# nianticlabs/implicit-depth

Hardware: AMD Instinct MI355X
Metric: frames/sec (BDModel.forward hot path, 512x384, 64 planes, 8-frame tuple = 1 current + 7 source views; third-party backbones excluded) (higher is better)
Workload: dtype f32

## Files before the change

### implicit-depth_amd/csrc/conv.hip

```cpp
#include <algorithm>
#include "conv_args.h"
#include "../../include/idh_ops.h"

using namespace idh_conv;

int idh_stem_op(const idh_op &op, hipStream_t st, bool launch);

namespace {

__device__ float g_zero_page[kZeroFloats];

thread_local bool t_dry_run = false;
thread_local int t_launches = 0;
#undef IDH_CHECK_LAUNCH
#define IDH_CHECK_LAUNCH()                                              \
    do {                                                                \
        if (!t_dry_run && hipGetLastError() != hipSuccess) return IDH_ELAUNCH; \
    } while (0)
#define IDH_LAUNCH(...)                         \
    do {                                        \
        if (t_dry_run) ++t_launches;            \
        else hipLaunchKernelGGL(__VA_ARGS__);   \
    } while (0)

// ... 1252 lines not shown
    } else {
        int tm = op.tile_m, tn = op.tile_n;
        if (tm == 8 || tm == 9) tm = 0;
        const int nsub = a.Cout_pad / 16;
        if (tn == 0) tn = (nsub % 4 == 0) ? 4 : (nsub % 2 == 0 ? 2 : 1);
        if (tm == 0) tm = 4;
        if ((tm != 1 && tm != 2 && tm != 4) || (tn != 1 && tn != 2 && tn != 4) || nsub % tn) return IDH_EINVAL;
        a.MT = (int)((M + 16 * tm - 1) / (16 * tm));
        a.NT = nsub / tn;
        pc.tm = tm; pc.tn = tn;
        const long long waves = (long long)a.MT * a.NT * a.S;
        if ((waves + 3) / 4 >= (1ll << 31)) return IDH_EUNSUPPORTED;
        pc.blocks = (unsigned)((waves + 3) / 4);
    }
    if (pc.up && ((pc.lds_rows != 8 && pc.lds_rows != 4) || pc.nj != 4)) return IDH_EUNSUPPORTED;
    if (pc.norm && ((pc.lds_rows != 8 && pc.lds_rows != 4) || pc.nj != 1)) return IDH_EUNSUPPORTED;
    if (a.S > 1) {
        if (!op.ws) return IDH_EWORKSPACE;
        pc.red = ReduceDesc{op.ws, op.bias, op.res, op.out, a.M, op.Cout, a.Cout_pad, a.S, op.res_cs, op.out_cs, op.act, op.slope};
    }
    return IDH_OK;
}

int launch_conv(const PreparedConv &pc, hipStream_t st) {
    if (pc.lds_rows == 16) {
        if (t_dry_run) { ++t_launches; return IDH_OK; }
        return launch_conv_split(pc.a, pc.n_img, pc.tm, pc.tn, st);
    }
    if (pc.lds_rows == 32) {
        if (t_dry_run) { ++t_launches; return IDH_OK; }
        return launch_conv_wino(pc.a, pc.n_img, pc.tn, st);
// ... 159 lines not shown
                    } else {
                        break;
                    }
                    ++run;
                }
                int cnt = 0;
                if (op.kind == IDH_OP_CONV && pcs[0].lds_rows == 4 && !pcs[0].norm && !pcs[0].s2) {
                    cnt = 1;
                    while (cnt < run && ops[i + cnt].kind == IDH_OP_CONV && pcs[cnt].lds_rows == 4 && pcs[cnt].nj == pcs[0].nj &&
                           (!pcs[cnt].up || pcs[0].nj == 4) && !pcs[cnt].norm && !pcs[cnt].s2)
                        ++cnt;
                }
                int mix = 0;
                while (mix < run && kinds[mix] >= 0 && pcs[mix].blocks <= kLevelMaxBlocks) ++mix;
                int wg = 0;
                if (op.kind == IDH_OP_CONV && pcs[0].lds_rows == 32) {
                    wg = 1;
                    while (wg < run && wg < wino_max_group() && ops[i + wg].kind == IDH_OP_CONV && pcs[wg].lds_rows == 32 &&
                           (pcs[wg].a.s[1].in != nullptr) == (pcs[0].a.s[1].in != nullptr))
                        ++wg;
                }
                int rc, used;
                if (wg > 1) {
                    if (t_dry_run) {
                        ++t_launches;
                        rc = IDH_OK;
                    } else {
                        const ConvArgs *as[kMaxGroup];
                        int ns[kMaxGroup];
                        for (int j = 0; j < wg; ++j) { as[j] = &pcs[j].a; ns[j] = pcs[j].n_img; }
                        rc = launch_conv_wino_group(as, ns, wg, st);
                        if (rc == IDH_EUNSUPPORTED) {
                            rc = IDH_OK;
// ... 176 lines not shown
```

### implicit-depth_amd/csrc/conv_wino.hip

```cpp
#include <type_traits>

#include "conv_args.h"
#include "../../include/idh_ops.h"

using namespace idh_conv;

namespace {

typedef unsigned u32x4_t __attribute__((ext_vector_type(4)));
typedef __attribute__((address_space(3))) void lds_void;

constexpr int kWinoCH = 8;
constexpr int kWinoTileW = 32;
constexpr int kWinoHalf = 17;
constexpr int kOob = 0x7fffffff;

constexpr int wino_plane(int WAVES) { return (2 * WAVES + 2) * 2 * kWinoHalf; }
constexpr int wino_qs(int WAVES) { return (wino_plane(WAVES) + 63) / 64 * 64; }
constexpr int wino_stage(int WAVES, int NCO) { return 4 * wino_qs(WAVES) + NCO * 1024; }

__global__ __launch_bounds__(256) void pack_wino_weight_k(const float *__restrict__ w, float *__restrict__ dst, int Cout, int Cin, int nS, int nCB, int KS) {
    const long long total = (long long)nS * nCB * 16 * 64 * KS;
    for (long long t = blockIdx.x * 256ll + threadIdx.x; t < total; t += gridDim.x * 256ll) {
        const int e = (int)(t % KS);
// ... 32 lines not shown
#endif

struct WinoArgs {
    ConvArgs c;
    int tiles_x, tiles_y;
    int tiles;
};

template <int WAVES, int NCO, int CH, bool SRC2>
constexpr int wino_stage_slots() {
    constexpr int halo = ((CH / 4) * wino_plane(WAVES) + 63) / 64 * 64;
    constexpr int s3 = halo + 64 * NCO * 4 * (CH / 4), sp = 8 * 32 * 2 * WAVES + 64 * 2 * NCO;
    return SRC2 && sp > s3 ? sp : s3;
}

template <int WAVES, int NCO, int CH, bool SRC2>
__device__ __forceinline__ void wino_tiles(const WinoArgs &wa, f32x4 *lds, const unsigned vblock, const unsigned vgrid) {
    constexpr int KS = CH / 4;
    constexpr int NP = CH / 4;
    typedef float vec __attribute__((ext_vector_type(KS)));
    constexpr int kRows = 2 * WAVES;
    constexpr int kPlane = wino_plane(WAVES);
    static_assert(NP == 2, "halo swizzle written for 8-channel K steps");
    constexpr int kHaloPieces = (NP * kPlane + 63) / 64;
    constexpr int kHP = (kHaloPieces + WAVES - 1) / WAVES;
    constexpr int kPanelPieces = NCO * 4 * KS;
    static_assert(kPanelPieces % WAVES == 0, "panel pieces must split evenly over the waves");
    constexpr int kPanel = kPanelPieces / WAVES;
    constexpr int kTPW = kHP + kPanel;
    static_assert(CH == 8, "K steps of 8 channels: every tile has >= 2 steps (the first stores the previous tile's outputs, the last loads the residual)");
    static_assert(kTPW <= 8 && 4 * NCO <= 8, "one DMA piece per even position group, one output store per odd group");
// ... 36 lines not shown
        unsigned blk = (unsigned)t;
        const int nt = blk % a.NT; blk /= a.NT;
        const int tx = blk % wa.tiles_x; blk /= wa.tiles_x;
        const int ty = blk % wa.tiles_y;
        img = blk / wa.tiles_y;
        y0 = ty * kRows; x0 = tx * kWinoTileW; cb0 = nt * NCO;
    };
    BufRef rsA;
    int voffH[kHP], panel_so;
    const int voffP = 16 * lane;
    auto halo_piece = [&](int k) { return wave + WAVES * k < kHaloPieces ? wave + WAVES * k : wave; };
    auto halo_voff = [&](int j, int lane) {
        const int pt = 32 * j + (lane >> 1);
        const int row = pt / kWinoHalf, hxh = pt - row * kWinoHalf;
        const int q = (lane & 1) ^ ((hxh >> 3) & 1);
        const int iy = y0 - 1 + (row >> 1), ix = x0 - 1 + 2 * hxh + (row & 1);
        const bool ok = (pt < kPlane) & ((unsigned)iy < (unsigned)s.H) & ((unsigned)ix < (unsigned)s.W);
        return ok ? (iy * s.W + ix) * s.cs * 4 + 16 * q : kOob;
    };
    auto set_fetch_tile = [&]() {
        rsA = BufRef{s.in + (size_t)img * s.H * s.W * s.cs, s.H * s.W * s.cs * 4};
        int lane_o = lane;
        asm volatile("" : "+v"(lane_o));
#pragma unroll
        for (int k = 0; k < kHP; ++k) voffH[k] = halo_voff(halo_piece(k), lane_o);
        panel_so = (cb0 * (4 * KS) + wave * kPanel) * 1024;
    };
    static_assert(!SRC2 || (kTight == 64 * WAVES && 2 * NCO == WAVES), "P-step pieces: eight of the pixels and one of the panel per wave");
    constexpr int kTPW2 = SRC2 ? 9 : 0;
    const ConvSrc &s1 = a.s[1];
    const int nS2 = SRC2 ? (s1.cblocks + 1) / 2 : 0;
// ... 42 lines not shown
                const int hh = wave / NCO, cbw = wave % NCO;
                halo1 = false;
                vo1 = voffP2; so1 = (4 * (2 * c + hh) * a.Cout_pad + 16 * (cbf + cbw)) * 16; lo1 = 8 * kTight + 64 * wave;
            }
            const int m = -(int)p;
            const unsigned long long m64 = (unsigned long long)(long long)m;
            vo ^= (vo ^ vo1) & m; so ^= (so ^ so1) & m; lo ^= (lo ^ lo1) & m;
            const BufRef rs1 = halo1 ? rsA2 : rsW2;
            const unsigned long long p0 = (unsigned long long)rs.p, p1 = (unsigned long long)rs1.p;
            rs.p = reinterpret_cast<const float *>(p0 ^ ((p0 ^ p1) & m64));
            rs.bytes ^= (rs.bytes ^ rs1.bytes) & m;
        }
        dma16(rs, lds + __builtin_amdgcn_readfirstlane(stage * kStage + lo), vo, __builtin_amdgcn_readfirstlane(so));
    };

    f32x4 acc[16][NCO];
    f32x4 ost[2][2][NCO];
    int voffS[2][2];
    __amdgpu_buffer_rsrc_t rsS;
    bool pending = false;

    const int pq = (KS * h) >> 2, pb8 = ((KS * h) & 3) * 4;
    const int patch0 = (NP * ((4 * wave) * kWinoHalf + n) + (pq ^ ((n >> 3) & 1))) * 16 + pb8;
    const int frag0 = kHalo * 16 + (h * 16 + n) * (4 * KS);

    constexpr int kAhead = CH == 16 ? 2 : 3;
    auto compute = [&](int stage, bool pnext, int cnext, int snext, int cbf, bool flush) {
        typedef const __attribute__((address_space(3))) volatile char lds_cchar;
        typedef const __attribute__((address_space(3))) volatile vec lds_cvec;
        int n_o = n;
        asm volatile("" : "+v"(n_o));
        const int patch1 = patch0 + (NP + ((pq ^ (((n_o + 1) >> 3) & 1)) - (pq ^ ((n_o >> 3) & 1)))) * 16;
        lds_cchar *sH0 = (lds_cchar *)(lds + stage * kStage) + patch0, *sH1 = (lds_cchar *)(lds + stage * kStage) + patch1;
        lds_cchar *sW = (lds_cchar *)(lds + stage * kStage) + frag0;
        vec d[4][4], A[kAhead + 1][NCO], r[4];
        auto rd_frag = [&](int g) {
            const int p = ((g >> 2) == 0 ? 4 : (g >> 2) == 1 ? 8 : (g >> 2) == 2 ? 0 : 12) + (g & 3);
#pragma unroll
            for (int j = 0; j < NCO; ++j) A[g % (kAhead + 1)][j] = *(lds_cvec *)(sW + (j * 16 + p) * 64 * (4 * KS));
        };
        auto rd_row = [&](int y) {
#pragma unroll
            for (int x = 0; x < 4; ++x) d[y][x] = *(lds_cvec *)(((x >> 1) ? sH1 : sH0) + NP * (2 * y + (x & 1)) * kWinoHalf * 16);
        };
        rd_frag(0);
        rd_row(1);
        rd_row(2);
#pragma unroll
        for (int g = 1; g < kAhead; ++g) rd_frag(g);
#pragma unroll
        for (int g = 0; g < 16; ++g) {
            const int xi = (g >> 2) == 0 ? 1 : (g >> 2) == 1 ? 2 : (g >> 2) == 2 ? 0 : 3, nu = g & 3;
            const int p = 4 * xi + nu;
            if (g + kAhead < 16) rd_frag(g + kAhead);
            if (g == 5) rd_row(0);
            if (g == 9) rd_row(3);
#ifndef IDH_ABL_WINO_NODMA
            if ((g & 1) == 0 && (g >> 1) < kTPW) issue_next(g >> 1, pnext, cnext, snext, cbf);
            if (SRC2 && (g == 1 || g == 3) && kTPW + (g >> 1) < kTPW2) {
// ... 2 lines not shown
#endif
#ifndef IDH_ABL_WINO_NOSTORE
            if ((g & 1) == 1 && (g >> 1) < 4 * NCO && flush) {
                const int k = g >> 1;
                __builtin_amdgcn_raw_buffer_store_b128(__builtin_bit_cast(u32x4_t, ost[k >> 1 & 1][k & 1][k >> 2]), rsS, voffS[k >> 1 & 1][k & 1] + 64 * (k >> 2), 0, 0);
            }
#endif
            __builtin_amdgcn_sched_barrier(0);
#ifdef IDH_ABL_WINO_SCALARXF
            auto vadd = [](vec a, vec b) { vec o; for (int e = 0; e < KS; ++e) { float t = a[e] + b[e]; asm("" : "+v"(t)); o[e] = t; } return o; };
            auto vsub = [](vec a, vec b) { vec o; for (int e = 0; e < KS; ++e) { float t = a[e] - b[e]; asm("" : "+v"(t)); o[e] = t; } return o; };
#else
            auto vadd = [](vec a, vec b) { return a + b; };
            auto vsub = [](vec a, vec b) { return a - b; };
#endif
#ifndef IDH_ABL_WINO_NOXFORM
            if (nu == 0) {
#pragma unroll
                for (int x = 0; x < 4; ++x)
                    r[x] = xi == 0 ? vsub(d[0][x], d[2][x]) : xi == 1 ? vadd(d[1][x], d[2][x]) : xi == 2 ? vsub(d[2][x], d[1][x]) : vsub(d[1][x], d[3][x]);
            }
#endif
#ifdef IDH_ABL_WINO_NOXFORM
            const vec v = d[xi][nu];
#else
            const vec v = nu == 0 ? vsub(r[0], r[2]) : nu == 1 ? vadd(r[1], r[2]) : nu == 2 ? vsub(r[2], r[1]) : vsub(r[1], r[3]);
#endif
#pragma unroll
            for (int k = 0; k < KS; ++k)
#pragma unroll
// ... 34 lines not shown
            const int px = g >> 1, hh = g & 1;
            const int pos = 12 * (px >> 1) + 3 * (px & 1);
            f32x4 bop = d2[px >> 1][px & 1][hh];
            if ((px >> 1) != (px & 1)) bop = -bop;
#pragma unroll
            for (int k = 0; k < 4; ++k)
#pragma unroll
                for (int j = 0; j < NCO; ++j)
                    acc[pos][j] = __builtin_amdgcn_mfma_f32_16x16x4f32(A1[hh][j][k], bop[k], acc[pos][j], 0, 0, 0);
            __builtin_amdgcn_sched_barrier(0);
        }
    };

    decode(t_cur);
    set_fetch_tile();
#pragma unroll
    for (int k = 0; k < kTPW; ++k) issue_next(k, false, 0, 0, 0);
    WINO_TRACE(tr_i++);
    asm volatile("s_waitcnt vmcnt(0)" ::: "memory");
    __syncthreads();
    WINO_TRACE(tr_i++);

    int it = 0;
#pragma unroll 1
    for (;;) {
        const int t_next = t_cur + t_stride;
        const bool has_next = t_next < t_end;
#pragma unroll
        for (int p = 0; p < 16; ++p)
#pragma unroll
// ... 19 lines not shown
#pragma unroll
                    for (int j = 0; j < 2; ++j) {
                        const int oy = y0 + 2 * wave + i, ox = x0 + 2 * n + j;
                        const bool ok = (oy < a.Ho) & (ox < a.Wo);
                        const int voffR = ok ? ((oy * a.Wo + ox) * a.res_cs + n0 + 4 * h) * 4 : kOob;
#pragma unroll
                        for (int cb = 0; cb < NCO; ++cb) ost[i][j][cb] = __builtin_bit_cast(f32x4, __builtin_amdgcn_raw_buffer_load_b128(rsR, voffR + 64 * cb, 0, 0));
                    }
#pragma unroll
                for (int cb = 0; cb < NCO; ++cb) b4[cb] = __builtin_bit_cast(f32x4, __builtin_amdgcn_raw_buffer_load_b128(rsB, (n0 + 16 * cb + 4 * h) * 4, 0, 0));
                if (has_next) {
                    decode(t_next);
                    set_fetch_tile();
                }
            }
            const bool pnext = SRC2 && !last && c + 1 >= nS;
            const int cnext = last ? 0 : pnext ? c + 1 - nS : c + 1, sn = (it + 1) & 1;
            if (!SRC2 || c < nS) {
                compute(it & 1, pnext, cnext, sn, cb_cur, pending);
                pending = false;
            } else {
                compute_p(it & 1, pnext, cnext, sn, cb_cur);
            }
            ++it;
            WINO_TRACE(tr_i < 61 ? tr_i++ : 61);
            asm volatile("s_waitcnt vmcnt(0)" ::: "memory");
            __syncthreads();
            WINO_TRACE(tr_i < 61 ? tr_i++ : 61);
        }

// ... 33 lines not shown
            }
        rsS = rsO;
        pending = true;
        WINO_TRACE(tr_i < 61 ? tr_i++ : 61);
        if (!has_next) break;
        t_cur = t_next;
    }
#ifndef IDH_ABL_WINO_NOSTORE
#pragma unroll
    for (int k = 0; k < 4 * NCO; ++k)
        __builtin_amdgcn_raw_buffer_store_b128(__builtin_bit_cast(u32x4_t, ost[k >> 1 & 1][k & 1][k >> 2]), rsS, voffS[k >> 1 & 1][k & 1] + 64 * (k >> 2), 0, 0);
#endif
    WINO_TRACE(62);
}

template <int WAVES, int NCO, int CH, bool SRC2>
__global__ __launch_bounds__(64 * WAVES, 2) void conv3x3_wino_k(const WinoArgs wa) {
    __shared__ f32x4 lds[2 * wino_stage_slots<WAVES, NCO, CH, SRC2>()];
    wino_tiles<WAVES, NCO, CH, SRC2>(wa, lds, blockIdx.x, gridDim.x);
}

constexpr int kWinoMaxGroup = 6;
struct WinoGroupArgs {
    WinoArgs op[kWinoMaxGroup];
    int rot[kWinoMaxGroup];
    int n;
};
template <int WAVES, int NCO, int CH, bool SRC2>
__global__ __launch_bounds__(64 * WAVES, 2) void conv3x3_wino_group_k(const WinoGroupArgs g) {
    __shared__ f32x4 lds[2 * wino_stage_slots<WAVES, NCO, CH, SRC2>()];
    const unsigned per = gridDim.x >> 3;
    for (int i = 0; i < g.n; ++i) {
        const unsigned vblock = (((blockIdx.x >> 3) + per - (unsigned)g.rot[i] % per) % per) << 3 | (blockIdx.x & 7);
        wino_tiles<WAVES, NCO, CH, SRC2>(g.op[i], lds, vblock, gridDim.x);
// ... 12 lines not shown
    return IDH_OK;
}

template <int WAVES, int NCO, int CH, bool SRC2>
long long wino_resident() {
    static int resident = 0;
    if (resident == 0) {
        int dev = 0, cus = 256;
        if (hipGetDevice(&dev) == hipSuccess) (void)hipDeviceGetAttribute(&cus, hipDeviceAttributeMultiprocessorCount, dev);
        resident = cus > 0 ? cus : 256;
    }
    constexpr int kLdsBytes = 2 * wino_stage_slots<WAVES, NCO, CH, SRC2>() * 16;
    return (long long)resident * (kLdsBytes * 2 <= 160 * 1024 ? 2 : 1);
}

template <int WAVES, int NCO, int CH, bool SRC2>
int launch_wino(const ConvArgs &a, int N, hipStream_t st) {
    WinoArgs wa;
    if (int rc = wino_args<WAVES, NCO>(a, N, wa)) return rc;
    long long grid = wino_resident<WAVES, NCO, CH, SRC2>();
    if (grid > wa.tiles) grid = wa.tiles >= 8 ? wa.tiles / 8 * 8 : wa.tiles;
    hipLaunchKernelGGL((conv3x3_wino_k<WAVES, NCO, CH, SRC2>), dim3((unsigned)grid), dim3(64 * WAVES), 0, st, wa);
    IDH_CHECK_LAUNCH();
    return IDH_OK;
}

template <int WAVES, int NCO, int CH, bool SRC2>
int launch_wino_group(const ConvArgs *const *as, const int *Ns, int n, hipStream_t st) {
    WinoGroupArgs g{};
    long long total = 0;
    int rot = 0;
    const long long res = wino_resident<WAVES, NCO, CH, SRC2>();
    for (int i = 0; i < n; ++i) {
        if (int rc = wino_args<WAVES, NCO>(*as[i], Ns[i], g.op[i])) return rc;
        g.rot[i] = rot;
        rot = (int)((rot + (g.op[i].tiles + 7) / 8) % (res / 8));
        total += g.op[i].tiles;
// ... 4 lines not shown
    if ((grid & 7) || (res & 7)) return IDH_EUNSUPPORTED;
    hipLaunchKernelGGL((conv3x3_wino_group_k<WAVES, NCO, CH, SRC2>), dim3((unsigned)grid), dim3(64 * WAVES), 0, st, g);
    IDH_CHECK_LAUNCH();
    return IDH_OK;
}

}

namespace idh_conv {

bool wino_supported(const ConvArgs &a) {
    const ConvSrc &s = a.s[0];
    const ConvSrc &s1 = a.s[1];
    const bool src2_ok = !s1.in || (s1.ks == 1 && s1.stride == 1 && !s1.up_in[0] && !s1.norm && s1.H == s.H && s1.W == s.W &&
                                    (long long)s1.H * s1.W * s1.cs * 4 < (1ll << 31) && (long long)s1.cblocks * a.Cout_pad * 64 < (1ll << 31));
    return s.ks == 3 && s.stride == 1 && s.pad_mode == IDH_PAD_ZEROS && !s.up_in[0] && !s.norm && src2_ok && a.S == 1 && (a.Cout % 32) == 0 &&
           (long long)s.H * s.W * s.cs * 4 < (1ll << 31) && (long long)a.Ho * a.Wo * a.out_cs * 4 < (1ll << 31) &&
           (!a.res || (long long)a.Ho * a.Wo * a.res_cs * 4 < (1ll << 31)) && (long long)s.cblocks * a.Cout_pad * 1024 < (1ll << 31);
}

int wino_max_group() { return kWinoMaxGroup; }

int launch_conv_wino_group(const ConvArgs *const *as, const int *Ns, int n, hipStream_t st) {
    if (n < 1 || n > kWinoMaxGroup) return IDH_EINVAL;
    const bool src2 = as[0]->s[1].in != nullptr;
    for (int i = 0; i < n; ++i)
        if (!wino_supported(*as[i]) || (as[i]->s[1].in != nullptr) != src2) return IDH_EUNSUPPORTED;
    return src2 ? launch_wino_group<4, 2, kWinoCH, true>(as, Ns, n, st) : launch_wino_group<4, 2, kWinoCH, false>(as, Ns, n, st);
}

int launch_conv_wino(const ConvArgs &a, int N, int rows, hipStream_t st) {
    if (!wino_supported(a)) return IDH_EUNSUPPORTED;
    (void)rows;
    return a.s[1].in ? launch_wino<4, 2, kWinoCH, true>(a, N, st) : launch_wino<4, 2, kWinoCH, false>(a, N, st);
}

}

extern "C" size_t idh_packed_wino_weight_floats(int Cout, int Cin) {
    if (Cout <= 0 || Cin <= 0) return 0;
    return (size_t)((Cin + 15) & ~15) * ((Cout + 15) & ~15) * 16;
}

extern "C" int idh_pack_conv_weight_wino(const float *w, float *dst, int Cout, int Cin, void *stream) {
    constexpr int ch = kWinoCH;
    if (!w || !dst || Cout <= 0 || Cin <= 0) return IDH_EINVAL;
    const int nC = (Cin + 15) / 16, nCB = (Cout + 15) / 16;
    const long long total = (long long)nC * nCB * 4096;
// ... 7 lines not shown
```

### implicit-depth_amd/csrc/networks.hip

```cpp
#include <algorithm>
#include <array>
#include <cstring>
#include <map>
#include <tuple>
#include <vector>

#include "idh_common.h"
#include "net_plan.h"
#include "../../include/idh_net.h"
#include "../../include/idh_ops.h"

namespace {

constexpr int kWinoMinTiles = 128;
constexpr double kWinoMinFill = 0.74;
constexpr int kWino4MinTiles = 768;
constexpr double kWino4MinFill = 0.85;
constexpr long long kReuseMinBytes = 64ll << 20;
constexpr int kNarrowTileBelow = 400;
constexpr int kSplitMinChunks = 6, kSplitMax = 16;
constexpr double kProjChunkWeight = 0.5;
constexpr int kS2FirstMinBlocks = 512;
constexpr int kTargetWaves = 2048, kMinWaves = 1024;
constexpr int kTileWino = IDH_TILE_WINO, kTileWino4 = IDH_TILE_WINO4;
constexpr bool kFuseHeadNorm = true;
constexpr bool kFuseHeadImport = true;

inline int ceil16(int v) { return (v + 15) & ~15; }
inline int cdiv(int a, int b) { return (a + b - 1) / b; }
inline size_t align64(size_t v) { return (v + 63) & ~(size_t)63; }

__global__ __launch_bounds__(256) void bias_sum_k(const float *__restrict__ a, const float *__restrict__ b, float *__restrict__ out, int n) {
    const int i = blockIdx.x * 256 + threadIdx.x;
    if (i < n) out[i] = (a ? a[i] : 0.f) + (b ? b[i] : 0.f);
}

enum Mode { MODE_SIZES, MODE_PACK, MODE_RUN };

struct Buf {
    float *base;
// ... 83 lines not shown
        b.N = n; b.H = t.H; b.W = t.W; b.cs = t.cs; b.internal = false; b.zero_fill = false;
        b.base = mode_ == MODE_RUN ? t.ptr : reinterpret_cast<float *>((uintptr_t(2) << 32) + ((uintptr_t)bufs.size() << 24));
        bufs.push_back(b);
        return View{(int)bufs.size() - 1, 0, t.C};
    }
    void release(const View &v) {
        const Buf &b = bufs[v.buf];
        if (!b.internal || v.c0 != 0 || v.C != b.cs || (long long)b.floats * 4 < kReuseMinBytes) return;
        auto &pool = free_[std::make_tuple(b.N, b.H, b.W, b.cs)];
        if (std::find(pool.begin(), pool.end(), v.buf) != pool.end()) { err = IDH_EINVAL; return; }
        pool.push_back(v.buf);
    }

    static Region region(const View &v, bool pad16 = false) { return Region{v.buf, v.c0, v.c0 + (pad16 ? ceil16(v.C) : v.C)}; }

    bool wino_eligible(const std::vector<Src> &srcs, int cout, int n, int Ho, int Wo, int pad_mode = IDH_PAD_ZEROS) const {
        const idh_conv_params &c0 = *srcs[0].cv;
        if (c0.ks != 3 || c0.stride != 1 || pad_mode != IDH_PAD_ZEROS || cout % 32) return false;
        if (srcs.size() > 1 && (srcs[1].cv->ks != 1 || srcs[1].cv->stride != 1)) return false;
        const int ty = cdiv(Ho, 8), tx = cdiv(Wo, 32);
        if ((double)Ho * Wo < kWinoMinFill * (ty * 8) * (tx * 32)) return false;
        return (long long)n * ty * tx * (cout / 32) >= kWinoMinTiles;
    }
    bool wino4_eligible(const std::vector<Src> &srcs, int cout, int n, int Ho, int Wo, int act, float slope, const View &out, const View *res,
                        int pad_mode = IDH_PAD_ZEROS, bool any_size = false) const {
        const idh_conv_params &c0 = *srcs[0].cv;
        const View &v0 = srcs[0].v;
        if (c0.ks != 3 || c0.stride != 1 || pad_mode != IDH_PAD_ZEROS || cout % 64) return false;
        if (srcs.size() > 1 && (srcs.size() > 2 || srcs[1].cv->ks != 1 || srcs[1].cv->stride != 1)) return false;
        if ((act != IDH_ACT_NONE && act != IDH_ACT_LRELU && act != IDH_ACT_ELU) || (act == IDH_ACT_LRELU && !(slope >= 0.f && slope <= 1.f)) || c0.cin <= 16) return false;
// ... 83 lines not shown
        }
        return dst;
    }

    View conv(const View &x, const idh_conv_params &cv, const View &out, int act, float slope, const View *res, const View *x2, const idh_conv_params *cv2,
              int pad_mode = IDH_PAD_ZEROS, const Norm *norm = nullptr, bool wino4_any_size = false) {
        if (err) return out;
        idh_op op;
        std::memset(&op, 0, sizeof op);
        op.kind = IDH_OP_CONV;
        op.N = N(x);
        std::vector<Src> srcs{{x, &cv}};
        if (x2) srcs.push_back({*x2, cv2});
        const int n = N(out), Ho = H(out), Wo = W(out), cout = cv.cout;
        if (out.C != cout) { err = IDH_EINVAL; return out; }
        bool use_wino = !norm && wino_eligible(srcs, cout, n, Ho, Wo, pad_mode);
        const bool use_wino4 = !norm && (!x2 || !res) && wino4_eligible(srcs, cout, n, Ho, Wo, act, slope, out, res, pad_mode, wino4_any_size);
        if (use_wino4) use_wino = false;
        int steps = 0;
        for (size_t i = 0; i < srcs.size(); ++i) {
            const View &v = srcs[i].v;
            const idh_conv_params &c = *srcs[i].cv;
            if (v.C != c.cin || (c.ks != 1 && c.ks != 3) || c.cout != cout) { err = IDH_EINVAL; return out; }
            if (v.C % 16 && (v.c0 != 0 || cs(v) != ceil16(v.C))) { err = IDH_EINVAL; return out; }
            const WLayout lay = (use_wino4 && i == 0) ? W_WINO4 : (use_wino && i == 0) ? W_WINO : W_DIRECT;
            idh_conv_src &s = op.src[i];
            s.in = ptr(v); s.w = packed(c, lay); s.cs = cs(v); s.H = H(v); s.W = W(v); s.Cin = v.C;
            s.ks = c.ks; s.stride = c.stride; s.pad_mode = pad_mode;
            steps += c.ks * c.ks * (ceil16(v.C) / 16);
        }
        op.bias = bias_of(cv, cv2);
// ... 12 lines not shown
            tn = lds_subtiles(cout);
            if (tn == 4 && tm == 9 && kNarrowTileBelow) {
                const long long blocks64 = (long long)n * cdiv(Ho, 4) * cdiv(Wo, 16) * (cout / 64) * split;
                if (blocks64 < kNarrowTileBelow) tn = 2;
            }
            tn = tn == 4 ? 0 : tn;
        } else if (!norm && s2_first_eligible(srcs, cout, n, Ho, Wo, pad_mode)) {
            choose_lds_tile(n, Ho, Wo, cout, ceil16(x.C) / 16, tm, split);
            tn = lds_subtiles(cout);
            tn = tn == 4 ? 0 : tn;
        } else {
            choose_tiles(M, cout, steps, tm, tn, split);
        }
        op.tile_m = tm; op.tile_n = tn; op.split_k = split;
        if (norm) {
            if ((tm != 8 && tm != 9) || tn != 1 || x2) { err = IDH_EINVAL; return out; }
            op.src[0].norm = norm->stats; op.src[0].norm_act = norm->act; op.src[0].norm_slope = norm->slope;
        }
        if (split > 1) op.ws = ws_alloc((size_t)split * M * ceil16(cout));
        ops.push_back(op);
        Meta m;
        if (res) m.reads.push_back(region(*res));
        if (norm) m.reads.push_back(Region{norm->buf, 0, 1});
        for (const Src &s : srcs) m.reads.push_back(region(s.v, true));
        m.writes.push_back(region(out));
        meta.push_back(m);
        return out;
    }
    void upsample2(const View &x, const View &out) {
        if (err) return;
        idh_op op;
// ... 570 lines not shown
```

### implicit-depth_amd/nhwc.py

```python
from __future__ import annotations

import ctypes as C
from dataclasses import dataclass
from typing import Dict, List, Optional, Sequence

import torch
from torch import nn

from . import _lib

OP_CONV, OP_UPSAMPLE2, OP_IMPORT, OP_EXPORT, OP_SPLITK, OP_HEAD, OP_INSTNORM, OP_UPSAMPLE2_NEAREST, OP_COPY, OP_POINTWISE_NCHW, OP_POINTWISE_UP = 1, 2, 3, 4, 5, 6, 7, 8, 9, 10, 11
OP_STEM = 12
ACT_NONE, ACT_LRELU, ACT_ELU = 0, 1, 2
PAD_ZEROS, PAD_REPLICATE = 0, 1


class ConvSrc(C.Structure):
    _fields_ = [("in_", C.c_void_p), ("w", C.c_void_p), ("cs", C.c_int32), ("H", C.c_int32), ("W", C.c_int32),
                ("Cin", C.c_int32), ("ks", C.c_int32), ("stride", C.c_int32), ("pad_mode", C.c_int32), ("_r", C.c_int32),
                ("up_in", C.c_void_p * 2), ("up_cs", C.c_int32 * 2), ("up_c0", C.c_int32), ("up_C", C.c_int32),
                ("norm", C.c_void_p), ("norm_slope", C.c_float), ("norm_act", C.c_int32)]


class Op(C.Structure):
# ... 129 lines not shown
    if (kh, kw) != (3, 3):
        raise _lib.IdhError("the Winograd F(4x4,3x3) kernel covers 3x3 convolutions only")
    dst = torch.empty(L.idh_packed_wino4_weight_floats(co, ci), device=w.device, dtype=torch.float32)
    wc = w.detach().contiguous()
    _lib.check(L.idh_pack_conv_weight_wino4(wc.data_ptr(), dst.data_ptr(), co, ci, _lib.stream_ptr()), "idh_pack_conv_weight_wino4")
    conv._idh_packed_wino4 = (key, dst)
    return dst


TILE_WINO = 12
TILE_WINO4 = 13
WINOGRAD = True
WINO_MIN_TILES = 128
WINO_MIN_FILL = 0.74
WINO_GROUP = True


def wino_eligible(srcs, cout: int, N: int, Ho: int, Wo: int, pad_mode: int) -> bool:
    (v0, c0) = srcs[0]
    if c0.kernel_size[0] != 3 or c0.stride[0] != 1 or pad_mode != PAD_ZEROS or cout % 32 or isinstance(v0, CatView):
        return False
    if len(srcs) > 1:
        (v1, c1) = srcs[1]
        if c1.kernel_size[0] != 1 or c1.stride[0] != 1 or isinstance(v1, CatView):
            return False
    ty, tx = -(-Ho // 8), -(-Wo // 32)
    if Ho * Wo < WINO_MIN_FILL * (ty * 8) * (tx * 32):
        return False
    return N * ty * tx * (cout // 32) >= WINO_MIN_TILES

# ... 84 lines not shown


def choose_split_rows(N: int, Ho: int, Wo: int, cout: int) -> int:
    def eff(rows, bonus):
        ty = -(-Ho // rows)
        blocks = N * ty * (-(-Wo // 16)) * (cout // 64)
        return bonus * (Ho / (ty * rows)) * min(1.0, blocks / 768.0)
    return 16 if Ho >= 16 and eff(16, 1.0) >= eff(8, 0.93) else 8


FUSE_UPSAMPLE = False
FUSED_UP_ROWS = 4

MERGE_LEVELS = True
FUSE_HEAD_NORM = True
FUSE_HEAD_IMPORT = True

TARGET_WAVES = 2048
MIN_WAVES = 1024


def lds_eligible(srcs, cout: int, Wo: int, pad_mode: int) -> bool:
    (v0, c0) = srcs[0]
    if c0.kernel_size[0] != 3 or c0.stride[0] != 1 or cout % 16 or Wo < 16:
        return False
    if pad_mode != PAD_ZEROS and (pad_mode != PAD_REPLICATE or len(srcs) > 1):
        return False
    if len(srcs) > 1:
        (v1, c1) = srcs[1]
        strided3 = c1.kernel_size[0] == 3 and c1.stride[0] == 2 and pad_mode == PAD_ZEROS and cout % 32 == 0 and not isinstance(v1, CatView)
# ... 88 lines not shown
                and any(t is k for k in self.keep)):
            pool = self._free.setdefault(tuple(t.shape), [])
            if any(t is f for f in pool):
                raise _lib.IdhError("Plan.release: buffer released twice")
            pool.append(t)
            self.recycled_candidates += 1

    def conv(self, x: View, conv: nn.Conv2d, out: View, act=ACT_NONE, slope=0.2, res: Optional[View] = None,
             x2: Optional[View] = None, conv2: Optional[nn.Conv2d] = None, pad_mode=PAD_ZEROS, norm=None, wino4_any_size: bool = False):
        op = Op()
        op.kind = OP_CONV
        op.N = x.N
        srcs = [(x, conv)] + ([(x2, conv2)] if x2 is not None else [])
        steps = 0
        use_split = self.math != "fp32" and split_eligible(srcs, conv.out_channels, out.N, out.H, out.W, pad_mode)
        use_wino = (WINOGRAD and self.math == "fp32" and norm is None and
                    wino_eligible(srcs, conv.out_channels, out.N, out.H, out.W, pad_mode))
        use_wino4 = (WINOGRAD4 and self.math == "fp32" and norm is None and (x2 is None or res is None) and
                     wino4_eligible(srcs, conv.out_channels, out.N, out.H, out.W, pad_mode, act, out, res, slope, wino4_any_size))
        if use_wino4:
            use_wino = False
        for i, (v, cv) in enumerate(srcs):
            ks, st = cv.kernel_size[0], cv.stride[0]
            if v.C != cv.in_channels:
                raise _lib.IdhError(f"conv expects {cv.in_channels} input channels, view has {v.C}")
            cat = v if isinstance(v, CatView) else None
            if cat is not None:
                if use_split or not lds_eligible(srcs, conv.out_channels, out.W, pad_mode) or st != 1:
                    raise _lib.IdhError("a fused-upsample concat can only feed the LDS-staged fp32 conv kernel")
                if cat.direct.C % 16 or any(u.C != cat.ups[0].C or u.C % 16 or (2 * u.H, 2 * u.W) != (cat.H, cat.W) for u in cat.ups) or not 1 <= len(cat.ups) <= 2:
                    raise _lib.IdhError("fused-upsample concat: channel counts must be multiples of 16 and the maps exactly half size")
                v = cat.direct
# ... 45 lines not shown
            tn = lds_subtiles(conv.out_channels)
            if tn == 4 and tm == 9 and NARROW_TILE_BELOW and not any(isinstance(v, CatView) for v, _ in srcs):
                blocks64 = out.N * (-(-out.H // 4)) * (-(-out.W // 16)) * (conv.out_channels // 64) * split
                if blocks64 < NARROW_TILE_BELOW:
                    tn = 1 if blocks64 < NARROWEST_TILE_BELOW else 2
            tn = 0 if tn == 4 else tn
        elif self.math == "fp32" and norm is None and s2_first_eligible(srcs, conv.out_channels, out.N, out.H, out.W, pad_mode):
            tm, split = choose_lds_tile(out.N, out.H, out.W, conv.out_channels, ceil16(x.C) // 16)
            tn = lds_subtiles(conv.out_channels)
            tn = 0 if tn == 4 else tn
        else:
            tm, tn, split = choose_tiles(M, conv.out_channels, steps)
        op.tile_m, op.tile_n, op.split_k = tm, tn, split
        if norm is not None:
            stats, n_act, n_slope = norm
            if tm not in (8, 9) or tn != 1 or x2 is not None or isinstance(x, CatView) or tuple(stats.shape) != (x.N, 2, x.C):
                raise _lib.IdhError("normalise-on-load needs the LDS-staged fp32 conv with 16-channel tiles and one source")
            op.src[0].norm, op.src[0].norm_act, op.src[0].norm_slope = stats.data_ptr(), n_act, n_slope
        if split > 1:
            ws = torch.empty(split * M * ceil16(conv.out_channels), device=self.device, dtype=torch.float32)
            self.keep.append(ws)
            op.ws = ws.data_ptr()
        self.ops.append(op)
        reads = ([_region(res)] if res is not None else []) + ([(norm[0].data_ptr(), 0, 1)] if norm is not None else [])
        for v, _ in srcs:
            if isinstance(v, CatView):
                reads += [_region(v.direct)] + [_region(u) for u in v.ups]
            else:
                reads.append(_region(v, pad16=True))
        self.meta.append({"reads": reads, "writes": [_region(out)]})
        self._arr = None
        return out
# ... 337 lines not shown
        return ent

    def values(self):
        return self.d.values()

    def __len__(self):
        return len(self.d)

    def clear(self):
        self.d.clear()


def build_flags() -> tuple:
    return (WINO_GROUP, FUSE_UPSAMPLE, FUSED_UP_ROWS, MERGE_LEVELS, FUSE_HEAD_NORM, FUSE_HEAD_IMPORT, NARROW_TILE_BELOW, NARROWEST_TILE_BELOW, SPLIT_MIN_CHUNKS,
            SPLIT_MAX, SPLIT_MIN_BLOCKS, WINOGRAD, WINO_MIN_TILES, WINO_MIN_FILL, WINOGRAD4, WINOGRAD4_PROJ, WINO4_MIN_TILES, WINO4_MIN_FILL, BUFFER_REUSE, REUSE_MIN_BYTES, DEFAULT_MATH,
            S2_FIRST, S2_FIRST_MIN_BLOCKS, PROJ_CHUNK_WEIGHT, PROJ_LOWRES, PROJ_LOWRES_MIN_TILES)


def _plan_cache(module: nn.Module) -> PlanCache:
    c = module.__dict__.get("_idh_plans")
    if c is None:
        c = PlanCache()
        module.__dict__["_idh_plans"] = c
        _lib.watch_state_dict_loads(module)
    return c


def _param_key(module: nn.Module):
    return ParamKey((math_of(module), build_flags()) + tuple((p.data_ptr(), _lib.param_version(p)) for p in module.parameters()))


# ... 443 lines not shown
```

Baseline: 680.6.

## Route replicate-padded head convs through Winograd kernel with fused normalise-on-load

Adds a replicate-padding variant of the F(2x2,3x3) Winograd conv kernel. It clamps halo coordinates instead of zero-filling, and it can apply per-image instance-norm statistics plus optional leaky-ReLU to the input tiles before the transform. Both the Python and C++ planners now send 3x3 stride-1 replicate-padded single-source head convs to this kernel, including normalised ones, instead of the LDS-staged direct conv. The variant uses NCO=1 and is excluded from grouped Winograd launches. The cost it targets is extra arithmetic in direct 3x3 convs. The trade-off is a new code path with per-K-step stats loads and narrower output tiles.

```diff
diff --git a/implicit-depth_amd/csrc/conv.hip b/implicit-depth_amd/csrc/conv.hip
--- a/implicit-depth_amd/csrc/conv.hip
+++ b/implicit-depth_amd/csrc/conv.hip
@@ -1290,7 +1290,7 @@
         pc.blocks = (unsigned)((waves + 3) / 4);
     }
     if (pc.up && ((pc.lds_rows != 8 && pc.lds_rows != 4) || pc.nj != 4)) return IDH_EUNSUPPORTED;
-    if (pc.norm && ((pc.lds_rows != 8 && pc.lds_rows != 4) || pc.nj != 1)) return IDH_EUNSUPPORTED;
+    if (pc.norm && pc.lds_rows != 32 && ((pc.lds_rows != 8 && pc.lds_rows != 4) || pc.nj != 1)) return IDH_EUNSUPPORTED;
     if (a.S > 1) {
         if (!op.ws) return IDH_EWORKSPACE;
         pc.red = ReduceDesc{op.ws, op.bias, op.res, op.out, a.M, op.Cout, a.Cout_pad, a.S, op.res_cs, op.out_cs, op.act, op.slope};
@@ -1480,9 +1480,9 @@
                 int mix = 0;
                 while (mix < run && kinds[mix] >= 0 && pcs[mix].blocks <= kLevelMaxBlocks) ++mix;
                 int wg = 0;
-                if (op.kind == IDH_OP_CONV && pcs[0].lds_rows == 32) {
+                if (op.kind == IDH_OP_CONV && pcs[0].lds_rows == 32 && pcs[0].a.s[0].pad_mode == IDH_PAD_ZEROS) {
                     wg = 1;
-                    while (wg < run && wg < wino_max_group() && ops[i + wg].kind == IDH_OP_CONV && pcs[wg].lds_rows == 32 &&
+                    while (wg < run && wg < wino_max_group() && ops[i + wg].kind == IDH_OP_CONV && pcs[wg].lds_rows == 32 && pcs[wg].a.s[0].pad_mode == IDH_PAD_ZEROS &&
                            (pcs[wg].a.s[1].in != nullptr) == (pcs[0].a.s[1].in != nullptr))
                         ++wg;
                 }
diff --git a/implicit-depth_amd/csrc/conv_wino.hip b/implicit-depth_amd/csrc/conv_wino.hip
--- a/implicit-depth_amd/csrc/conv_wino.hip
+++ b/implicit-depth_amd/csrc/conv_wino.hip
@@ -70,7 +70,7 @@
     return SRC2 && sp > s3 ? sp : s3;
 }
 
-template <int WAVES, int NCO, int CH, bool SRC2>
+template <int WAVES, int NCO, int CH, bool SRC2, bool REP = false>
 __device__ __forceinline__ void wino_tiles(const WinoArgs &wa, f32x4 *lds, const unsigned vblock, const unsigned vgrid) {
     constexpr int KS = CH / 4;
     constexpr int NP = CH / 4;
@@ -137,7 +137,11 @@
         const int pt = 32 * j + (lane >> 1);
         const int row = pt / kWinoHalf, hxh = pt - row * kWinoHalf;
         const int q = (lane & 1) ^ ((hxh >> 3) & 1);
-        const int iy = y0 - 1 + (row >> 1), ix = x0 - 1 + 2 * hxh + (row & 1);
+        int iy = y0 - 1 + (row >> 1), ix = x0 - 1 + 2 * hxh + (row & 1);
+        if constexpr (REP) {
+            iy = min(max(iy, 0), s.H - 1);
+            ix = min(max(ix, 0), s.W - 1);
+        }
         const bool ok = (pt < kPlane) & ((unsigned)iy < (unsigned)s.H) & ((unsigned)ix < (unsigned)s.W);
         return ok ? (iy * s.W + ix) * s.cs * 4 + 16 * q : kOob;
     };
@@ -210,6 +214,21 @@
         dma16(rs, lds + __builtin_amdgcn_readfirstlane(stage * kStage + lo), vo, __builtin_amdgcn_readfirstlane(so));
     };
 
+    static_assert(!REP || (!SRC2 && KS == 2), "replicate-padded variant: one source, 8-channel K steps");
+    const float nslope = REP && s.norm && s.norm_act == IDH_ACT_LRELU ? s.norm_slope : 1.f;
+    vec nm = {}, nr = {}, nm1 = {}, nr1 = {};
+    auto load_stats = [&](int im, int c) {
+        if constexpr (REP) {
+            nm1 = (vec){0.f, 0.f};
+            nr1 = (vec){1.f, 1.f};
+            if (s.norm) {
+                const float *st = s.norm + (size_t)im * 2 * s.Cin + CH * c + KS * h;
+                nm1 = *reinterpret_cast<const vec *>(st);
+                nr1 = *reinterpret_cast<const vec *>(st + s.Cin);
+            }
+        }
+    };
+
     f32x4 acc[16][NCO];
     f32x4 ost[2][2][NCO];
     int voffS[2][2];
@@ -239,6 +258,17 @@
 #pragma unroll
             for (int x = 0; x < 4; ++x) d[y][x] = *(lds_cvec *)(((x >> 1) ? sH1 : sH0) + NP * (2 * y + (x & 1)) * kWinoHalf * 16);
         };
+        auto norm_row = [&](int y) {
+            if constexpr (REP) {
+#pragma unroll
+                for (int x = 0; x < 4; ++x)
+#pragma unroll
+                    for (int e = 0; e < KS; ++e) {
+                        const float t = (d[y][x][e] - nm[e]) * nr[e];
+                        d[y][x][e] = fmaxf(t, t * nslope);
+                    }
+            }
+        };
         rd_frag(0);
         rd_row(1);
         rd_row(2);
@@ -271,6 +301,9 @@
             auto vadd = [](vec a, vec b) { return a + b; };
             auto vsub = [](vec a, vec b) { return a - b; };
 #endif
+            if (g == 0) { norm_row(1); norm_row(2); }
+            if (g == 7) norm_row(0);
+            if (g == 11) norm_row(3);
 #ifndef IDH_ABL_WINO_NOXFORM
             if (nu == 0) {
 #pragma unroll
@@ -335,6 +368,7 @@
 
     decode(t_cur);
     set_fetch_tile();
+    load_stats(img, 0);
 #pragma unroll
     for (int k = 0; k < kTPW; ++k) issue_next(k, false, 0, 0, 0);
     WINO_TRACE(tr_i++);
@@ -384,6 +418,11 @@
                     set_fetch_tile();
                 }
             }
+            if constexpr (REP) {
+                nm = nm1;
+                nr = nr1;
+                load_stats(img, last ? 0 : c + 1);
+            }
             const bool pnext = SRC2 && !last && c + 1 >= nS;
             const int cnext = last ? 0 : pnext ? c + 1 - nS : c + 1, sn = (it + 1) & 1;
             if (!SRC2 || c < nS) {
@@ -447,10 +486,10 @@
     WINO_TRACE(62);
 }
 
-template <int WAVES, int NCO, int CH, bool SRC2>
+template <int WAVES, int NCO, int CH, bool SRC2, bool REP = false>
 __global__ __launch_bounds__(64 * WAVES, 2) void conv3x3_wino_k(const WinoArgs wa) {
     __shared__ f32x4 lds[2 * wino_stage_slots<WAVES, NCO, CH, SRC2>()];
-    wino_tiles<WAVES, NCO, CH, SRC2>(wa, lds, blockIdx.x, gridDim.x);
+    wino_tiles<WAVES, NCO, CH, SRC2, REP>(wa, lds, blockIdx.x, gridDim.x);
 }
 
 constexpr int kWinoMaxGroup = 6;
@@ -493,13 +532,13 @@
     return (long long)resident * (kLdsBytes * 2 <= 160 * 1024 ? 2 : 1);
 }
 
-template <int WAVES, int NCO, int CH, bool SRC2>
+template <int WAVES, int NCO, int CH, bool SRC2, bool REP = false>
 int launch_wino(const ConvArgs &a, int N, hipStream_t st) {
     WinoArgs wa;
     if (int rc = wino_args<WAVES, NCO>(a, N, wa)) return rc;
     long long grid = wino_resident<WAVES, NCO, CH, SRC2>();
     if (grid > wa.tiles) grid = wa.tiles >= 8 ? wa.tiles / 8 * 8 : wa.tiles;
-    hipLaunchKernelGGL((conv3x3_wino_k<WAVES, NCO, CH, SRC2>), dim3((unsigned)grid), dim3(64 * WAVES), 0, st, wa);
+    hipLaunchKernelGGL((conv3x3_wino_k<WAVES, NCO, CH, SRC2, REP>), dim3((unsigned)grid), dim3(64 * WAVES), 0, st, wa);
     IDH_CHECK_LAUNCH();
     return IDH_OK;
 }
@@ -534,7 +573,10 @@
     const ConvSrc &s1 = a.s[1];
     const bool src2_ok = !s1.in || (s1.ks == 1 && s1.stride == 1 && !s1.up_in[0] && !s1.norm && s1.H == s.H && s1.W == s.W &&
                                     (long long)s1.H * s1.W * s1.cs * 4 < (1ll << 31) && (long long)s1.cblocks * a.Cout_pad * 64 < (1ll << 31));
-    return s.ks == 3 && s.stride == 1 && s.pad_mode == IDH_PAD_ZEROS && !s.up_in[0] && !s.norm && src2_ok && a.S == 1 && (a.Cout % 32) == 0 &&
+    const bool rep_ok = s.pad_mode == IDH_PAD_REPLICATE && !s1.in && (a.Cout % 16) == 0 && (s.Cin % 16) == 0 &&
+                        (!s.norm || s.norm_act == IDH_ACT_NONE || (s.norm_act == IDH_ACT_LRELU && s.norm_slope >= 0.f && s.norm_slope <= 1.f));
+    const bool zeros_ok = s.pad_mode == IDH_PAD_ZEROS && !s.norm && src2_ok && (a.Cout % 32) == 0;
+    return s.ks == 3 && s.stride == 1 && (zeros_ok || rep_ok) && !s.up_in[0] && a.S == 1 &&
            (long long)s.H * s.W * s.cs * 4 < (1ll << 31) && (long long)a.Ho * a.Wo * a.out_cs * 4 < (1ll << 31) &&
            (!a.res || (long long)a.Ho * a.Wo * a.res_cs * 4 < (1ll << 31)) && (long long)s.cblocks * a.Cout_pad * 1024 < (1ll << 31);
 }
@@ -545,13 +587,14 @@
     if (n < 1 || n > kWinoMaxGroup) return IDH_EINVAL;
     const bool src2 = as[0]->s[1].in != nullptr;
     for (int i = 0; i < n; ++i)
-        if (!wino_supported(*as[i]) || (as[i]->s[1].in != nullptr) != src2) return IDH_EUNSUPPORTED;
+        if (!wino_supported(*as[i]) || as[i]->s[0].pad_mode != IDH_PAD_ZEROS || (as[i]->s[1].in != nullptr) != src2) return IDH_EUNSUPPORTED;
     return src2 ? launch_wino_group<4, 2, kWinoCH, true>(as, Ns, n, st) : launch_wino_group<4, 2, kWinoCH, false>(as, Ns, n, st);
 }
 
 int launch_conv_wino(const ConvArgs &a, int N, int rows, hipStream_t st) {
     if (!wino_supported(a)) return IDH_EUNSUPPORTED;
     (void)rows;
+    if (a.s[0].pad_mode == IDH_PAD_REPLICATE) return launch_wino<4, 1, kWinoCH, false, true>(a, N, st);
     return a.s[1].in ? launch_wino<4, 2, kWinoCH, true>(a, N, st) : launch_wino<4, 2, kWinoCH, false>(a, N, st);
 }
 
diff --git a/implicit-depth_amd/csrc/networks.hip b/implicit-depth_amd/csrc/networks.hip
--- a/implicit-depth_amd/csrc/networks.hip
+++ b/implicit-depth_amd/csrc/networks.hip
@@ -24,6 +24,7 @@
 constexpr int kTargetWaves = 2048, kMinWaves = 1024;
 constexpr int kTileWino = IDH_TILE_WINO, kTileWino4 = IDH_TILE_WINO4;
 constexpr bool kFuseHeadNorm = true;
+constexpr bool kHeadWino = true;
 constexpr bool kFuseHeadImport = true;
 
 inline int ceil16(int v) { return (v + 15) & ~15; }
@@ -137,6 +138,12 @@
 
     static Region region(const View &v, bool pad16 = false) { return Region{v.buf, v.c0, v.c0 + (pad16 ? ceil16(v.C) : v.C)}; }
 
+    bool head_wino_eligible(const std::vector<Src> &srcs, int cout, int pad_mode, const Norm *norm) const {
+        const idh_conv_params &c0 = *srcs[0].cv;
+        if (!kHeadWino || pad_mode != IDH_PAD_REPLICATE || srcs.size() > 1) return false;
+        if (c0.ks != 3 || c0.stride != 1 || cout % 16 || srcs[0].v.C % 16) return false;
+        return !norm || norm->act == IDH_ACT_NONE || (norm->act == IDH_ACT_LRELU && norm->slope >= 0.f && norm->slope <= 1.f);
+    }
     bool wino_eligible(const std::vector<Src> &srcs, int cout, int n, int Ho, int Wo, int pad_mode = IDH_PAD_ZEROS) const {
         const idh_conv_params &c0 = *srcs[0].cv;
         if (c0.ks != 3 || c0.stride != 1 || pad_mode != IDH_PAD_ZEROS || cout % 32) return false;
@@ -250,7 +257,7 @@
         if (x2) srcs.push_back({*x2, cv2});
         const int n = N(out), Ho = H(out), Wo = W(out), cout = cv.cout;
         if (out.C != cout) { err = IDH_EINVAL; return out; }
-        bool use_wino = !norm && wino_eligible(srcs, cout, n, Ho, Wo, pad_mode);
+        bool use_wino = (!norm && wino_eligible(srcs, cout, n, Ho, Wo, pad_mode)) || head_wino_eligible(srcs, cout, pad_mode, norm);
         const bool use_wino4 = !norm && (!x2 || !res) && wino4_eligible(srcs, cout, n, Ho, Wo, act, slope, out, res, pad_mode, wino4_any_size);
         if (use_wino4) use_wino = false;
         int steps = 0;
@@ -293,7 +300,7 @@
         }
         op.tile_m = tm; op.tile_n = tn; op.split_k = split;
         if (norm) {
-            if ((tm != 8 && tm != 9) || tn != 1 || x2) { err = IDH_EINVAL; return out; }
+            if (!(((tm == 8 || tm == 9) && tn == 1) || tm == kTileWino) || x2) { err = IDH_EINVAL; return out; }
             op.src[0].norm = norm->stats; op.src[0].norm_act = norm->act; op.src[0].norm_slope = norm->slope;
         }
         if (split > 1) op.ws = ws_alloc((size_t)split * M * ceil16(cout));
diff --git a/implicit-depth_amd/nhwc.py b/implicit-depth_amd/nhwc.py
--- a/implicit-depth_amd/nhwc.py
+++ b/implicit-depth_amd/nhwc.py
@@ -167,6 +167,15 @@
 WINO_MIN_TILES = 128
 WINO_MIN_FILL = 0.74
 WINO_GROUP = True
+
+
+def head_wino_eligible(srcs, cout: int, pad_mode: int, norm=None) -> bool:
+    (v0, c0) = srcs[0]
+    if not HEAD_WINO or pad_mode != PAD_REPLICATE or len(srcs) > 1 or isinstance(v0, CatView):
+        return False
+    if c0.kernel_size[0] != 3 or c0.stride[0] != 1 or cout % 16 or v0.C % 16:
+        return False
+    return norm is None or norm[1] == ACT_NONE or (norm[1] == ACT_LRELU and 0.0 <= norm[2] <= 1.0)
 
 
 def wino_eligible(srcs, cout: int, N: int, Ho: int, Wo: int, pad_mode: int) -> bool:
@@ -281,6 +290,7 @@
 
 MERGE_LEVELS = True
 FUSE_HEAD_NORM = True
+HEAD_WINO = True
 FUSE_HEAD_IMPORT = True
 
 TARGET_WAVES = 2048
@@ -399,8 +409,8 @@
         srcs = [(x, conv)] + ([(x2, conv2)] if x2 is not None else [])
         steps = 0
         use_split = self.math != "fp32" and split_eligible(srcs, conv.out_channels, out.N, out.H, out.W, pad_mode)
-        use_wino = (WINOGRAD and self.math == "fp32" and norm is None and
-                    wino_eligible(srcs, conv.out_channels, out.N, out.H, out.W, pad_mode))
+        use_wino = self.math == "fp32" and ((WINOGRAD and norm is None and wino_eligible(srcs, conv.out_channels, out.N, out.H, out.W, pad_mode)) or
+                                            head_wino_eligible(srcs, conv.out_channels, pad_mode, norm))
         use_wino4 = (WINOGRAD4 and self.math == "fp32" and norm is None and (x2 is None or res is None) and
                      wino4_eligible(srcs, conv.out_channels, out.N, out.H, out.W, pad_mode, act, out, res, slope, wino4_any_size))
         if use_wino4:
@@ -476,8 +486,8 @@
         op.tile_m, op.tile_n, op.split_k = tm, tn, split
         if norm is not None:
             stats, n_act, n_slope = norm
-            if tm not in (8, 9) or tn != 1 or x2 is not None or isinstance(x, CatView) or tuple(stats.shape) != (x.N, 2, x.C):
-                raise _lib.IdhError("normalise-on-load needs the LDS-staged fp32 conv with 16-channel tiles and one source")
+            if not (tm in (8, 9) and tn == 1 or tm == TILE_WINO) or x2 is not None or isinstance(x, CatView) or tuple(stats.shape) != (x.N, 2, x.C):
+                raise _lib.IdhError("normalise-on-load needs the LDS-staged fp32 conv with 16-channel tiles (or the replicate-padded Winograd kernel) and one source")
             op.src[0].norm, op.src[0].norm_act, op.src[0].norm_slope = stats.data_ptr(), n_act, n_slope
         if split > 1:
             ws = torch.empty(split * M * ceil16(conv.out_channels), device=self.device, dtype=torch.float32)
@@ -845,7 +855,7 @@
 def build_flags() -> tuple:
     return (WINO_GROUP, FUSE_UPSAMPLE, FUSED_UP_ROWS, MERGE_LEVELS, FUSE_HEAD_NORM, FUSE_HEAD_IMPORT, NARROW_TILE_BELOW, NARROWEST_TILE_BELOW, SPLIT_MIN_CHUNKS,
             SPLIT_MAX, SPLIT_MIN_BLOCKS, WINOGRAD, WINO_MIN_TILES, WINO_MIN_FILL, WINOGRAD4, WINOGRAD4_PROJ, WINO4_MIN_TILES, WINO4_MIN_FILL, BUFFER_REUSE, REUSE_MIN_BYTES, DEFAULT_MATH,
-            S2_FIRST, S2_FIRST_MIN_BLOCKS, PROJ_CHUNK_WEIGHT, PROJ_LOWRES, PROJ_LOWRES_MIN_TILES)
+            S2_FIRST, S2_FIRST_MIN_BLOCKS, PROJ_CHUNK_WEIGHT, PROJ_LOWRES, PROJ_LOWRES_MIN_TILES, HEAD_WINO)
 
 
 def _plan_cache(module: nn.Module) -> PlanCache:
```

New measurement: 684.7, median of 6. No clear change (+0.6%).
